# yflyl613/Tiny-NewsRec

Hardware: AMD Instinct MI355X
Metric: training impressions/sec (higher is better)
Workload: dtype fp16; 1 GPU; Tiny-NewsRec 4-layer student (train [2, 3]) + 4-teacher KD (title-emb MSE + soft-CE), fwd+bwd+AMSGrad; batch_per_gpu=32, global_batch=32, user_log_length=50, candidates=5, num_words_title=30, news_dim=256, n_news=51282, parallelism=dp1

## Files before the change

tiny-newsrec_amd/csrc/heads.hip:

```cpp
#include "common.h"

namespace {

__global__ __launch_bounds__(256) void attpool_long_score_kernel(const float* __restrict__ e, int64_t lde, const float* __restrict__ w2,
                                                                 const float* __restrict__ b2, int Q, float* __restrict__ alpha,
                                                                 int64_t n_tok, int L) {
    const int lane = threadIdx.x & 63;
    const int64_t t = (int64_t)blockIdx.x * 4 + (threadIdx.x >> 6);
    if (t >= n_tok) return;
    const float* er = e + t * lde;
    float s = 0.f;
    for (int q = lane; q < Q; q += 64) s += er[q] * w2[q];
    s = wave_sum(s);
    const int Lr = (L + 31) & ~31;
    if (lane == 0) alpha[(t / L) * Lr + (t % L)] = __expf(s + b2[0]);
}
__global__ __launch_bounds__(256) void attpool_long_fwd_fin_kernel(const float* __restrict__ ws, float* __restrict__ alpha,
                                                                   float* __restrict__ nv, float* __restrict__ den, int L, int H) {
    __shared__ float dsh, al[512];
    const int Lr = (L + 31) & ~31, nch = (L + AP_CH - 1) / AP_CH;
    const int64_t n = blockIdx.x;
    for (int i = threadIdx.x; i < L; i += 256) al[i] = alpha[n * Lr + i];
    __syncthreads();
    if (threadIdx.x == 0) {
        float d = 0.f;
        for (int i = 0; i < L; ++i) d += al[i];
        dsh = d + 1e-8f;
        den[n] = d + 1e-8f;
    }
    __syncthreads();
    const float d = dsh;
    for (int c = threadIdx.x * 4; c < H; c += 1024) {
        f32x4 a = *(const f32x4*)(ws + (n * nch) * H + c);
        for (int ch = 1; ch < nch; ++ch) a += *(const f32x4*)(ws + (n * nch + ch) * H + c);
        *(f32x4*)(nv + n * H + c) = a / d;
    }
    for (int i = threadIdx.x; i < Lr; i += 256) alpha[n * Lr + i] = i < L ? al[i] / d : 0.f;
}
__global__ __launch_bounds__(256) void attpool_long_bwd_fin_kernel(const float* __restrict__ part, int Q, int64_t lddpre, int nch,
                                                                   float* __restrict__ dw2_part, float* __restrict__ db2_part,
                                                                   float* __restrict__ db1_part) {
    const int64_t n = blockIdx.x;
    const int64_t W = Q + lddpre + 1;
    for (int64_t j = threadIdx.x; j < W; j += 256) {
        float s = part[(n * nch) * W + j];
        for (int ch = 1; ch < nch; ++ch) s += part[(n * nch + ch) * W + j];
        if (j < Q) dw2_part[n * Q + j] = s;
        else if (j < Q + lddpre) { if (db1_part) db1_part[n * lddpre + (j - Q)] = s; }
        else db2_part[n] = s;
    }
}

struct SgemmArgs {
    const float* A; int64_t a_rs, a_cs, sA;
    const float* B; int64_t b_rs, b_cs, sB;
    float* C; int64_t ldc, sC;
    const float* bias; int64_t sBias;
    int M, N, K;
    float alpha, beta;
    int ksplit, kchunk, batch;
    float* A_out;
};

constexpr int SG_BK = 64;
__device__ __forceinline__ void sgemm_tile(const SgemmArgs& g, int bx, int by, int bz, float (&As)[64][SG_BK + 1], float (&Bs)[64][SG_BK + 1]) {
    const int tid = threadIdx.x, lane = tid & 63, w = tid >> 6, wm = w >> 1, wn = w & 1;
    const int zb = bz / g.ksplit, zk = bz - zb * g.ksplit;
    const float* A = g.A + zb * g.sA;
    const float* B = g.B + zb * g.sB;
    float* C = g.ksplit > 1 ? g.C + ((int64_t)zk * g.batch + zb) * g.M * g.N : g.C + zb * g.sC;
    const int64_t ldc = g.ksplit > 1 ? g.N : g.ldc;
    const int m0 = by * 64, n0 = bx * 64;
    const int kbeg = zk * g.kchunk;
    const int kend = kbeg + g.kchunk < g.K ? kbeg + g.kchunk : g.K;
    f32x16 acc;
#pragma unroll
    for (int r = 0; r < 16; ++r) acc[r] = 0.f;
    const bool a_kfast = g.a_cs == 1, b_kfast = g.b_cs == 1;
    constexpr int NQ = 64 * SG_BK / 256;
    const int ra0 = a_kfast ? tid >> 6 : tid & 63, ka0 = a_kfast ? tid & 63 : tid >> 6;
    const int rb0 = b_kfast ? tid >> 6 : tid & 63, kb0 = b_kfast ? tid & 63 : tid >> 6;
    float av[NQ], bv[NQ];
    auto fetch = [&](int k0) {
#pragma unroll
        for (int q = 0; q < NQ; ++q) {
            const int ra = a_kfast ? ra0 + 4 * q : ra0, ka = a_kfast ? ka0 : ka0 + 4 * q;
            const int rb = b_kfast ? rb0 + 4 * q : rb0, kb = b_kfast ? kb0 : kb0 + 4 * q;
            av[q] = (m0 + ra < g.M && k0 + ka < kend) ? A[(int64_t)(m0 + ra) * g.a_rs + (int64_t)(k0 + ka) * g.a_cs] : 0.f;
            bv[q] = (n0 + rb < g.N && k0 + kb < kend) ? B[(int64_t)(n0 + rb) * g.b_rs + (int64_t)(k0 + kb) * g.b_cs] : 0.f;
        }
    };
    fetch(kbeg);
    for (int k0 = kbeg; k0 < kend; k0 += SG_BK) {
#pragma unroll
        for (int q = 0; q < NQ; ++q) {
            const int ra = a_kfast ? ra0 + 4 * q : ra0, ka = a_kfast ? ka0 : ka0 + 4 * q;
            const int rb = b_kfast ? rb0 + 4 * q : rb0, kb = b_kfast ? kb0 : kb0 + 4 * q;
            As[ra][ka] = av[q];
            Bs[rb][kb] = bv[q];
        }
        __syncthreads();
        if (k0 + SG_BK < kend) fetch(k0 + SG_BK);
        const int kk_end = kend - k0 < SG_BK ? kend - k0 : SG_BK;
        for (int kk = 0; kk < kk_end; kk += 2) {
            float a = As[wm * 32 + (lane & 31)][kk + (lane >> 5)];
            float b = Bs[wn * 32 + (lane & 31)][kk + (lane >> 5)];
            acc = __builtin_amdgcn_mfma_f32_32x32x2f32(a, b, acc, 0, 0, 0);
        }
        __syncthreads();
    }
    const int n = n0 + wn * 32 + (lane & 31);
    if (n >= g.N) return;
    const float bias = (g.bias && g.ksplit == 1) ? g.bias[zb * g.sBias + n] : 0.f;
#pragma unroll
    for (int r = 0; r < 16; ++r) {
        int m = m0 + wm * 32 + (r & 3) + 8 * (r >> 2) + 4 * (lane >> 5);
        if (m < g.M) {
            float* c = C + (int64_t)m * ldc + n;
            if (g.ksplit > 1) {
                *c = acc[r];
            } else {
                float v = g.alpha * acc[r] + bias;
                if (g.beta != 0.f) v += g.beta * *c;
                *c = v;
            }
        }
    }
}

__global__ __launch_bounds__(256) void sgemm_kernel(SgemmArgs g) {
    __shared__ float As[64][SG_BK + 1], Bs[64][SG_BK + 1];
    sgemm_tile(g, blockIdx.x, blockIdx.y, blockIdx.z, As, Bs);
}

constexpr int SG_MAXP = 8;
struct SgemmGroup {
    SgemmArgs a[SG_MAXP];
    int start[SG_MAXP + 1];
    int gx[SG_MAXP], gy[SG_MAXP];
    int64_t rstart[SG_MAXP + 1];
    float alpha[SG_MAXP], beta[SG_MAXP];
    int n;
};
__global__ __launch_bounds__(256) void sgemm_group_kernel(SgemmGroup g) {
    __shared__ float As[64][SG_BK + 1], Bs[64][SG_BK + 1];
    const int b = blockIdx.x;
    int i = 0;
#pragma unroll
    for (int k = 1; k < SG_MAXP; ++k)
        if (k < g.n && b >= g.start[k]) i = k;
    const int l = b - g.start[i];
    const int per = g.gx[i] * g.gy[i];
    const int bz = l / per, r = l - bz * per;
    const int by = r / g.gx[i], bx = r - by * g.gx[i];
    sgemm_tile(g.a[i], bx, by, bz, As, Bs);
}
__global__ __launch_bounds__(256) void sgemm_group_reduce_kernel(SgemmGroup g) {
    const int64_t e = (int64_t)blockIdx.x * blockDim.x + threadIdx.x;
    if (e >= g.rstart[g.n]) return;
    int i = 0;
#pragma unroll
    for (int k = 1; k < SG_MAXP; ++k)
        if (k < g.n && e >= g.rstart[k]) i = k;
    const SgemmArgs& a = g.a[i];
    const int64_t per = (int64_t)a.M * a.N, total = per * a.batch, j = e - g.rstart[i];
    const float* part = a.C;
    float t = part[j];
    for (int s = 1; s < a.ksplit; ++s) t += part[(int64_t)s * total + j];
    const int z = (int)(j / per);
    const int64_t rr = j - (int64_t)z * per;
    const int m = (int)(rr / a.N), n = (int)(rr - (int64_t)m * a.N);
    float* c = (float*)a.A_out + (int64_t)z * a.sC + (int64_t)m * a.ldc + n;
    float v = g.alpha[i] * t + (a.bias ? a.bias[(int64_t)z * a.sBias + n] : 0.f);
    if (g.beta[i] != 0.f) v += g.beta[i] * *c;
    *c = v;
}

__global__ __launch_bounds__(256) void sgemm_reduce_kernel(const float* __restrict__ part, int ksplit, int batch, int M, int N,
                                                           float* __restrict__ C, int64_t ldc, int64_t sC,
                                                           const float* __restrict__ bias, int64_t sBias, float alpha, float beta) {
    const int64_t per = (int64_t)M * N, total = per * batch;
    const int64_t i = (int64_t)blockIdx.x * blockDim.x + threadIdx.x;
    if (i >= total) return;
    float t = part[i];
    for (int s = 1; s < ksplit; ++s) t += part[(int64_t)s * total + i];
    const int z = (int)(i / per);
    const int64_t r = i - (int64_t)z * per;
    const int m = (int)(r / N), n = (int)(r - (int64_t)m * N);
    float* c = C + (int64_t)z * sC + (int64_t)m * ldc + n;
    float v = alpha * t + (bias ? bias[(int64_t)z * sBias + n] : 0.f);
    if (beta != 0.f) v += beta * *c;
    *c = v;
}

__global__ void gather_rows_kernel(const float* __restrict__ tbl, int64_t R, const int32_t* __restrict__ idx,
                                   int64_t n_idx, int D, float* __restrict__ out, int64_t out_rows, int64_t out_row0) {
    int64_t t = (int64_t)blockIdx.x * blockDim.x + threadIdx.x;
    int d4 = D / 4;
    int64_t total = n_idx * d4;
    if (t >= total) return;
    int z = blockIdx.y;
    int64_t r = t / d4;
    int c = (int)(t - r * d4) * 4;
    *(f32x4*)(out + ((int64_t)z * out_rows + out_row0 + r) * D + c) =
        *(const f32x4*)(tbl + ((int64_t)z * R + idx[r]) * D + c);
}


__global__ __launch_bounds__(1024) void segment_sum_rows_kernel(const float* __restrict__ src, const int32_t* __restrict__ order,
                                                                const int32_t* __restrict__ seg, int D, float* __restrict__ out) {
    extern __shared__ __attribute__((aligned(16))) float sm[];
    const int u = blockIdx.x, lane = threadIdx.x & 63, w = threadIdx.x >> 6;
    const int j0 = seg[u], j1 = seg[u + 1];
    if (j1 - j0 <= 4) {
        if (w == 0)
            for (int c = lane * 4; c < D; c += 256) {
                f32x4 a = (f32x4){0.f, 0.f, 0.f, 0.f};
                for (int j = j0; j < j1; ++j) a += *(const f32x4*)(src + (int64_t)order[j] * D + c);
                *(f32x4*)(out + (int64_t)u * D + c) = a;
            }
        return;
    }
    for (int c = lane * 4; c < D; c += 256) {
        f32x4 a[4];
#pragma unroll
        for (int q = 0; q < 4; ++q) a[q] = (f32x4){0.f, 0.f, 0.f, 0.f};
        int j = j0 + w;
        for (; j + 48 < j1; j += 64) {
// ... 635 lines not shown
    if (threadIdx.x == 0) {
        losses[0] = red[0][0] / (float)B;
        losses[1] = red[1][0] / (float)B;
    }
}

__global__ __launch_bounds__(256) void kd_embed_loss_kernel(const float* __restrict__ S, const float* __restrict__ P,
                                                            const float* __restrict__ tw, float* __restrict__ dS,
                                                            float* __restrict__ dP, float* __restrict__ part, int B,
                                                            int U, int C, int D, int T) {
    const int lane = threadIdx.x & 63;
    const int64_t wv = (int64_t)blockIdx.x * 4 + (threadIdx.x >> 6);
    const int64_t nh = (int64_t)B * U, nn = (int64_t)B * (U + C), rtot = nn + B;
    if (wv >= rtot) return;
    int b;
    float rowscale;
    if (wv < nh) { b = (int)(wv / U); rowscale = 1.f / (float)(U + C); }
    else if (wv < nn) { b = (int)((wv - nh) / C); rowscale = 1.f / (float)(U + C); }
    else { b = (int)(wv - nn); rowscale = 1.f; }
    float loss = 0.f;
    for (int c = lane * 4; c < D; c += 256) {
        f32x4 s = *(const f32x4*)(S + wv * D + c);
        f32x4 g = (f32x4){0.f, 0.f, 0.f, 0.f};
        for (int i = 0; i < T; ++i) {
            float wi = tw[(int64_t)b * T + i];
            float ci = wi * rowscale * 2.f / ((float)D * (float)B);
            int64_t off = ((int64_t)i * rtot + wv) * D + c;
            f32x4 df = s - *(const f32x4*)(P + off);
            loss += wi * rowscale * (df[0] * df[0] + df[1] * df[1] + df[2] * df[2] + df[3] * df[3]);
            g += ci * df;
            *(f32x4*)(dP + off) = -ci * df;
        }
        *(f32x4*)(dS + wv * D + c) = g;
    }
    loss = wave_sum(loss);
    if (lane == 0) part[wv] = loss / ((float)D * (float)B);
}

__global__ __launch_bounds__(256) void score_bwd_kernel(const float* __restrict__ vec, const int32_t* __restrict__ cidx,
                                                        const float* __restrict__ user, const float* __restrict__ dscore,
                                                        float* __restrict__ dvec, float* __restrict__ duser, int C, int D) {
    const int b = blockIdx.x;
    for (int d = threadIdx.x; d < D; d += 256) {
        float u = user[(int64_t)b * D + d], acc = 0.f;
        for (int c = 0; c < C; ++c) {
            float g = dscore[(int64_t)b * C + c];
            int64_t row = cidx[(int64_t)b * C + c];
            acc += g * vec[row * D + d];
            dvec[row * D + d] += g * u;
        }
        duser[(int64_t)b * D + d] += acc;
    }
}

}

void attpool_long_score_launch(const float* e, int64_t lde, const float* w2, const float* b2, int Q, float* alpha, int64_t n_tok,
                               int L, hipStream_t st) {
    hipLaunchKernelGGL(attpool_long_score_kernel, dim3((unsigned)((n_tok + 3) / 4)), dim3(256), 0, st, e, lde, w2, b2, Q, alpha, n_tok, L);
}
void attpool_long_fwd_fin_launch(const float* ws, float* alpha, float* nv, float* den, int64_t n_seq, int L, int H, hipStream_t st) {
    hipLaunchKernelGGL(attpool_long_fwd_fin_kernel, dim3((unsigned)n_seq), dim3(256), 0, st, ws, alpha, nv, den, L, H);
}
void attpool_long_bwd_fin_launch(const float* part, int Q, int64_t lddpre, int nch, float* dw2_part, float* db2_part,
                                 float* db1_part, int64_t n_seq, hipStream_t st) {
    hipLaunchKernelGGL(attpool_long_bwd_fin_kernel, dim3((unsigned)n_seq), dim3(256), 0, st, part, Q, lddpre, nch, dw2_part,
                       db2_part, db1_part);
}

extern "C" int tnr_sgemm(const float* A, int64_t a_rs, int64_t a_cs, int64_t sA, const int32_t* a_idx, const float* B,
                         int64_t b_rs, int64_t b_cs, int64_t sB, float* C, int64_t ldc, int64_t sC, const float* bias,
                         int64_t sBias, int64_t M, int64_t N, int64_t K, int batch, float alpha, float beta,
                         int ksplit, float* part, void* stream) {
    TNR_CHECK_ARG(A && B && C && M >= 1 && N >= 1 && K >= 1 && batch >= 1, "tnr_sgemm: bad argument");
    TNR_CHECK_ARG(a_idx == nullptr, "tnr_sgemm: row gather is done by tnr_gather_rows");
    if (ksplit < 1) ksplit = 1;
    int kchunk = (int)K;
    if (ksplit > 1) {
        TNR_CHECK_ARG(part != nullptr, "tnr_sgemm: split-K needs the partial buffer (ksplit * batch * M * N floats)");
        kchunk = (int)(((K + ksplit - 1) / ksplit + 15) / 16 * 16);
        ksplit = (int)((K + kchunk - 1) / kchunk);
    }
    SgemmArgs g{A, a_rs, a_cs, sA, B, b_rs, b_cs, sB, ksplit > 1 ? part : C, ldc, sC, bias, sBias, (int)M, (int)N, (int)K,
                alpha, ksplit > 1 ? 0.f : beta, ksplit, kchunk, batch, C};
    dim3 grid((unsigned)((N + 63) / 64), (unsigned)((M + 63) / 64), (unsigned)(batch * ksplit));
    hipLaunchKernelGGL(sgemm_kernel, grid, dim3(256), 0, (hipStream_t)stream, g);
    TNR_CHECK_LAUNCH("tnr_sgemm");
    if (ksplit > 1) {
        const int64_t total = (int64_t)batch * M * N;
        hipLaunchKernelGGL(sgemm_reduce_kernel, dim3((unsigned)((total + 255) / 256)), dim3(256), 0, (hipStream_t)stream, part,
                           ksplit, batch, (int)M, (int)N, C, ldc, sC, bias, sBias, alpha, beta);
        TNR_CHECK_LAUNCH("tnr_sgemm/reduce");
    }
    return TNR_OK;
}

extern "C" int tnr_sgemm_group(const tnr_sgemm_problem_t* p, int n, void* stream) {
    TNR_CHECK_ARG(p && n >= 1 && n <= SG_MAXP, "tnr_sgemm_group: 1..%d problems", SG_MAXP);
    SgemmGroup g;
    g.n = n;
    g.start[0] = 0;
    g.rstart[0] = 0;
    for (int i = 0; i < n; ++i) {
        const tnr_sgemm_problem_t& q = p[i];
        TNR_CHECK_ARG(q.A && q.B && q.C && q.M >= 1 && q.N >= 1 && q.K >= 1 && q.batch >= 1, "tnr_sgemm_group: bad problem %d", i);
        int ksplit = q.ksplit < 1 ? 1 : q.ksplit;
        int kchunk = (int)q.K;
        if (ksplit > 1) {
            TNR_CHECK_ARG(q.part != nullptr, "tnr_sgemm_group: split-K needs the partial buffer (problem %d)", i);
            kchunk = (int)(((q.K + ksplit - 1) / ksplit + 15) / 16 * 16);
            ksplit = (int)((q.K + kchunk - 1) / kchunk);
        }
        g.a[i] = SgemmArgs{q.A, q.a_rs, q.a_cs, q.sA, q.B, q.b_rs, q.b_cs, q.sB, ksplit > 1 ? q.part : q.C, q.ldc, q.sC, q.bias, q.sBias,
                           (int)q.M, (int)q.N, (int)q.K, q.alpha, ksplit > 1 ? 0.f : q.beta, ksplit, kchunk, q.batch, q.C};
        g.gx[i] = (int)((q.N + 63) / 64);
        g.gy[i] = (int)((q.M + 63) / 64);
        g.start[i + 1] = g.start[i] + g.gx[i] * g.gy[i] * q.batch * ksplit;
        g.rstart[i + 1] = g.rstart[i] + (ksplit > 1 ? (int64_t)q.batch * q.M * q.N : 0);
        g.alpha[i] = q.alpha;
        g.beta[i] = q.beta;
    }
    for (int i = n; i < SG_MAXP; ++i) { g.start[i + 1] = g.start[n]; g.rstart[i + 1] = g.rstart[n]; g.gx[i] = g.gy[i] = 1; g.a[i] = g.a[0]; g.alpha[i] = g.beta[i] = 0.f; }
    hipLaunchKernelGGL(sgemm_group_kernel, dim3((unsigned)g.start[n]), dim3(256), 0, (hipStream_t)stream, g);
    TNR_CHECK_LAUNCH("tnr_sgemm_group");
    if (g.rstart[n] > 0) {
        hipLaunchKernelGGL(sgemm_group_reduce_kernel, dim3((unsigned)((g.rstart[n] + 255) / 256)), dim3(256), 0, (hipStream_t)stream, g);
        TNR_CHECK_LAUNCH("tnr_sgemm_group/reduce");
    }
    return TNR_OK;
}

__global__ __launch_bounds__(256) void concat_i32_kernel(const int32_t* __restrict__ a, int64_t na, const int32_t* __restrict__ b,
                                                         int64_t nb, int32_t* __restrict__ out) {
    const int64_t i = (int64_t)blockIdx.x * blockDim.x + threadIdx.x;
    if (i < na) out[i] = a[i];
    else if (i < na + nb) out[i] = b[i - na];
}

extern "C" int tnr_concat_i32(const int32_t* a, int64_t na, const int32_t* b, int64_t nb, int32_t* out, void* stream) {
    TNR_CHECK_ARG(out && na >= 0 && nb >= 0 && na + nb >= 1 && (a || na == 0) && (b || nb == 0), "tnr_concat_i32: bad argument");
    hipLaunchKernelGGL(concat_i32_kernel, dim3((unsigned)((na + nb + 255) / 256)), dim3(256), 0, (hipStream_t)stream, a, na, b, nb, out);
    TNR_CHECK_LAUNCH("tnr_concat_i32");
    return TNR_OK;
}

extern "C" int tnr_gather_rows(const float* tbl, int64_t R, const int32_t* idx, int64_t n_idx, int D, int n_model,
                               float* out, int64_t out_rows, int64_t out_row0, void* stream) {
    TNR_CHECK_ARG(tbl && idx && out && n_idx >= 1 && (D % 4) == 0 && n_model >= 1, "tnr_gather_rows: bad argument");
    int64_t total = n_idx * (D / 4);
    dim3 grid((unsigned)((total + 255) / 256), (unsigned)n_model);
    hipLaunchKernelGGL(gather_rows_kernel, grid, dim3(256), 0, (hipStream_t)stream, tbl, R, idx, n_idx, D, out, out_rows,
                       out_row0);
    TNR_CHECK_LAUNCH("tnr_gather_rows");
    return TNR_OK;
}

extern "C" int tnr_segment_sum_rows(const float* src, const int32_t* order, const int32_t* seg, int64_t n_seg, int D,
                                    float* out, void* stream) {
    TNR_CHECK_ARG(src && order && seg && out && n_seg >= 1 && D >= 4 && (D % 4) == 0 && D <= 2048,
                  "tnr_segment_sum_rows: bad argument");
    hipLaunchKernelGGL(segment_sum_rows_kernel, dim3((unsigned)n_seg), dim3(1024), 16 * D * sizeof(float),
                       (hipStream_t)stream, src, order, seg, D, out);
    TNR_CHECK_LAUNCH("tnr_segment_sum_rows");
    return TNR_OK;
}

extern "C" int tnr_scatter_sum_rows(const float* src, int64_t n, int D, const int32_t* keys_sorted, const int32_t* order,
                                    int32_t skip_key, float* table, int64_t table_rows, int accumulate, void* stream) {
    TNR_CHECK_ARG(src && keys_sorted && order && table && n >= 1 && n <= 0x7FFFFFFF && table_rows >= 1 && D >= 4 && (D % 4) == 0 &&
                  D <= 2048, "tnr_scatter_sum_rows: bad argument");
    hipLaunchKernelGGL(scatter_sum_rows_kernel, dim3((unsigned)n), dim3(1024), 16 * D * sizeof(float), (hipStream_t)stream, src, n,
                       D, keys_sorted, order, skip_key, table, table_rows, accumulate);
    TNR_CHECK_LAUNCH("tnr_scatter_sum_rows");
    return TNR_OK;
}

static int user_shape_ok(int B, int U, int C, int D, int Q) {
    return B >= 1 && U >= 1 && U <= MAXU && C >= 0 && (D % 4) == 0 && D >= 4 && Q >= 4 && (Q % 4) == 0;
}

extern "C" int tnr_user_score_fwd(const float* vec, int64_t R, const int32_t* hidx, const int32_t* cidx,
                                  const float* mask, const float* pad, const float* w1, const float* b1, const float* w2,
                                  const float* b2, int user_log_mask, const float* epre, const float* epad, float* user,
                                  int64_t user_stride,
                                  float* score, float* e, float* alpha, float* den, int n_model, int B, int U, int C, int D,
                                  int Q, void* stream) {
    TNR_CHECK_ARG(vec && hidx && cidx && mask && pad && w1 && b1 && w2 && b2 && user && score && e && alpha && den,
                  "tnr_user_score_fwd: null pointer");
    TNR_CHECK_ARG(user_shape_ok(B, U, C, D, Q) && n_model >= 1 && user_stride >= (int64_t)B * D,
                  "tnr_user_score_fwd: bad shape (U <= %d)", MAXU);
    if (!epre) {
        size_t lf = sizeof(float) * ((size_t)64 * (D + UF_XTRA) + (size_t)U * Q + MAXU + D);
        TNR_CHECK_ARG((D % 8) == 0 && lf <= 160 * 1024, "tnr_user_score_fwd: fused fc1 needs D %% 8 == 0 and 64 (D + 4) + U Q floats of LDS");
        TNR_ONCE_PER_DEVICE({
            (void)hipFuncSetAttribute((const void*)user_fwd_fused_kernel, hipFuncAttributeMaxDynamicSharedMemorySize, 160 * 1024);
        });
        hipLaunchKernelGGL(user_fwd_fused_kernel, dim3((unsigned)B, (unsigned)n_model), dim3(UF_THREADS), lf, (hipStream_t)stream,
// ... 133 lines not shown
```

tiny-newsrec_amd/csrc/testhooks.hip:

```cpp
#include "common.h"

namespace {
__global__ __launch_bounds__(1024) void cu_hog_kernel(unsigned long long ticks) {
    extern __shared__ char hog_lds[];
    if (threadIdx.x == 0) hog_lds[0] = 1;
    const unsigned long long t0 = __builtin_amdgcn_s_memrealtime();
    while (__builtin_amdgcn_s_memrealtime() - t0 < ticks) __builtin_amdgcn_s_sleep(64);
}
}

void tnr_set_error(const char*, ...) {}

extern "C" int tnr_debug_cu_hog(int n_wg, int us, void* stream) {
    if (!(n_wg >= 1 && n_wg <= 1024 && us >= 0 && us <= 100000)) return TNR_EINVAL;
    TNR_ONCE_PER_DEVICE({ (void)hipFuncSetAttribute((const void*)cu_hog_kernel, hipFuncAttributeMaxDynamicSharedMemorySize, 160 * 1024); });
    hipLaunchKernelGGL(cu_hog_kernel, dim3((unsigned)n_wg), dim3(1024), 160 * 1024, (hipStream_t)stream, (unsigned long long)us * 100ull);
    return hipGetLastError() == hipSuccess ? TNR_OK : TNR_ELAUNCH;
}
```

tiny-newsrec_amd/tnr_hip.py:

```python
import ctypes
import os

import torch

_HERE = os.path.dirname(os.path.abspath(__file__))
LIB_PATH = os.path.join(_HERE, "csrc", "libtnr_hip.so")

BF16, F16, F32 = 0, 1, 2
ROUTE_128, ROUTE_256x128, ROUTE_256, ROUTE_224 = 128, 2128, 256, 224
EPI_BIAS, EPI_GELU, EPI_TANH, EPI_RES, EPI_MULDGELU, EPI_OUTF32, EPI_AUXOUT, EPI_COLSUM = 1, 2, 4, 8, 16, 32, 64, 128

_c = ctypes
_P, _I, _L, _F = _c.c_void_p, _c.c_int, _c.c_int64, _c.c_float

DROP_EMB, DROP_PROB, DROP_ATTN_OUT, DROP_FFN_OUT = 0, 1, 2, 3


class Dropout(_c.Structure):
    _fields_ = [("seed", _c.c_uint64), ("site", _c.c_uint32), ("call", _c.c_uint32), ("p", _c.c_double)]

    @classmethod
    def site_of(cls, p, seed, kind, layer, call):
        if p is None or p <= 0.0:
            return None
# ... 91 lines not shown
    "tnr_attn_l32_bwd": [_P, _P, _P, _P, _P, _P, _L, _I, _I, _P],
    "tnr_attn_long_fwd": [_P, _P, _P, _P, _P, _L, _I, _I, _P],
    "tnr_attn_long_bwd": [_P, _P, _P, _P, _P, _P, _P, _P, _L, _I, _I, _P],
    "tnr_colsum": [_P, _L, _I, _L, _L, _P, _P, _I, _P],
    "tnr_colsum_batched": [_P, _L, _L, _I, _L, _L, _I, _P, _P, _I, _P],
    "tnr_colsum_part_elems": [_L, _L],
    "tnr_attpool_fwd": [_P, _P, _L, _P, _P, _I, _P, _P, _P, _L, _I, _I, _P],
    "tnr_attpool_bwd": [_P, _P, _L, _P, _I, _P, _P, _P, _P, _P, _L, _P, _P, _P, _L, _I, _I, _P],
    "tnr_attpool_fwd_long": [_P, _P, _L, _P, _P, _I, _P, _P, _P, _P, _L, _I, _I, _P],
    "tnr_attpool_bwd_long": [_P, _P, _L, _P, _I, _P, _P, _P, _P, _L, _P, _P, _P, _P, _L, _I, _I, _P],
    "tnr_sgemm": [_P, _L, _L, _L, _P, _P, _L, _L, _L, _P, _L, _L, _P, _L, _L, _L, _L, _I, _F, _F, _I, _P, _P],
    "tnr_sgemm_group": [_c.POINTER(SgemmProblem), _I, _P],
    "tnr_gemm_tn_wgrad_group": [_c.POINTER(WgradProblem), _I, _P],
    "tnr_concat_i32": [_P, _L, _P, _L, _P, _P],
    "tnr_gather_rows": [_P, _L, _P, _L, _I, _I, _P, _L, _L, _P],
    "tnr_segment_sum_rows": [_P, _P, _P, _L, _I, _P, _P],
    "tnr_scatter_sum_rows": [_P, _L, _I, _P, _P, _I, _P, _L, _I, _P],
    "tnr_user_score_fwd": [_P, _L, _P, _P, _P, _P, _P, _P, _P, _P, _I, _P, _P, _P, _L, _P, _P, _P, _P, _I, _I, _I, _I, _I, _I, _P],
    "tnr_user_bwd_pre": [_P, _P, _P, _P, _P, _I, _P, _P, _P, _P, _P, _P, _I, _I, _I, _I, _P],
    "tnr_user_bwd_post": [_P, _P, _P, _P, _P, _I, _P, _P, _I, _I, _I, _I, _P],
    "tnr_user_bwd_part_stride": [_I, _I],
    "tnr_user_blend_fwd": [_P, _L, _P, _P, _P, _I, _P, _I, _I, _I, _I, _P],
    "tnr_user_blend_bwd": [_P, _P, _P, _I, _P, _P, _L, _I, _I, _I, _P],
    "tnr_nrms_attn_fwd": [_P, _P, _I, _P, _L, _I, _I, _I, _I, _P],
    "tnr_nrms_attn_bwd": [_P, _P, _I, _P, _P, _I, _I, _I, _P],
    "tnr_score_bwd": [_P, _P, _P, _P, _P, _P, _I, _I, _I, _P],
    "tnr_kd_score_loss": [_P, _P, _P, _F, _F, _P, _P, _P, _I, _I, _I, _P],
    "tnr_kd_embed_loss": [_P, _P, _P, _P, _P, _P, _P, _I, _I, _I, _I, _I, _P],
    "tnr_reduce_rows": [_P, _L, _L, _L, _P, _I, _P],
    "tnr_reduce_multi": [_P, _I, _P],
    "tnr_dropout_mask": [_D, _L, _L, _P, _P],
    "tnr_dropout_mask_probs": [_D, _L, _I, _I, _P, _P],
    "tnr_dropout_mask_split": [_D, _D, _L, _L, _L, _P, _P],
    "tnr_scale_inplace": [_P, _L, _F, _P],
    "tnr_amsgrad_step": [_P, _P, _P, _P, _P, _L, _I, _F, _F, _F, _F, _F, _P],
    "tnr_amsgrad_step_guarded": [_P, _P, _P, _P, _P, _L, _I, _F, _F, _F, _F, _F, _P, _c.c_uint, _c.c_uint, _P],
    "tnr_grad_nonfinite": [_P, _L, _P, _c.c_uint, _P],
    "tnr_grad_nonfinite_scan": [_P, _L, _P, _c.c_uint, _P],
    "tnr_grad_nonfinite_commit": [_P, _c.c_uint, _P],
    "tnr_refresh_shadows": [_P, _I, _L, _P, _P],
    "tnr_cast_f32_to_bf16": [_P, _P, _L, _P],
    "tnr_cast_bf16_to_f32": [_P, _P, _L, _P],
}
TYPED = ["tnr_embed_ln_fwd", "tnr_embed_ln_fwd_indexed", "tnr_embed_ln_bwd", "tnr_embed_ln_bwd_indexed", "tnr_gemm_nt", "tnr_gemm_nt_ex", "tnr_gemm_colsum_rows", "tnr_gemm_nt_route",
         "tnr_gemm_tn_wgrad", "tnr_gemm_tn_wgrad_ex", "tnr_gemm_tn_wgrad_group", "tnr_gemm_tn_ws_elems", "tnr_ln_fwd", "tnr_ln_bwd", "tnr_attn_l32_fwd", "tnr_attn_l32_bwd", "tnr_attn_long_fwd", "tnr_attn_long_bwd",
         "tnr_colsum", "tnr_colsum_batched", "tnr_attpool_fwd", "tnr_attpool_bwd", "tnr_attpool_fwd_long", "tnr_attpool_bwd_long", "tnr_attpool_long_ws_elems", "tnr_refresh_shadows",
         "tnr_cast_f32_to_bf16", "tnr_cast_bf16_to_f32", "tnr_pool_fwd", "tnr_pool_bwd"]
for _n in ("tnr_embed_ln_fwd", "tnr_embed_ln_fwd_indexed", "tnr_attn_l32_fwd", "tnr_attn_l32_bwd", "tnr_attn_long_fwd", "tnr_attn_long_bwd"):
    _SIG[_n + "_do"] = _SIG[_n][:-1] + [_D] + ([_P] if "embed" in _n else []) + [_P]
    TYPED.append(_n + "_do")
_SIG["tnr_gemm_nt_do"] = _SIG["tnr_gemm_nt_ex"][:-1] + [_D, _P]
_SIG["tnr_ln_bwd_do"] = _SIG["tnr_ln_bwd"][:-1] + [_P, _D, _P]
_SIG["tnr_gemm_nt_do_split"] = _SIG["tnr_gemm_nt_do"][:-1] + [_D, _L, _P]
_SIG["tnr_ln_bwd_do_split"] = _SIG["tnr_ln_bwd_do"][:-1] + [_D, _L, _P]
TYPED += ["tnr_gemm_nt_do", "tnr_ln_bwd_do", "tnr_gemm_nt_do_split", "tnr_ln_bwd_do_split"]
for _n in TYPED:
    _SIG[_n + "_f16"] = _SIG[_n]
_RET = {"tnr_attpool_long_ws_elems": _L, "tnr_attpool_long_ws_elems_f16": _L, "tnr_gemm_tn_ws_elems": _L, "tnr_gemm_tn_ws_elems_f16": _L, "tnr_gemm_colsum_rows_f16": _L, "tnr_gemm_colsum_rows": _L, "tnr_ln_bwd_part_elems": _L, "tnr_ln_bwd_blocks": _L, "tnr_embed_ln_bwd_part_elems": _L, "tnr_embed_ln_bwd_blocks": _L, "tnr_colsum_part_elems": _L,
        "tnr_user_bwd_part_stride": _L}
EXPORTS = sorted(_SIG) + ["tnr_last_error"]

_lib = None


class TnrError(RuntimeError):
    pass


def lib():
    global _lib
    if _lib is None:
        if not os.path.exists(LIB_PATH):
            raise TnrError("libtnr_hip.so not built: run `make -C tiny-newsrec_amd/csrc` (or __graft_entry__.build())")
        L = ctypes.CDLL(LIB_PATH)
        for name, args in _SIG.items():
            fn = getattr(L, name)
            fn.argtypes = args
            fn.restype = _RET.get(name, _I)
        L.tnr_last_error.restype = ctypes.c_char_p
        _lib = L
    return _lib


def _ptr(t):
    if t is None:
        return None
    if isinstance(t, int):
        return t
    return t.data_ptr()


def _conv(a):
    if isinstance(a, Dropout):
        return ctypes.byref(a)
    return _ptr(a) if (isinstance(a, torch.Tensor) or a is None) else a


_raw_stream = getattr(torch._C, "_cuda_getCurrentRawStream", None)


def stream():
    if _raw_stream is not None:
        return _raw_stream(torch.cuda.current_device())
    return torch.cuda.current_stream().cuda_stream


TIMED = {}
TIMED_ALL = None


def _all_begin():
    if TIMED_ALL is None:
        return None
    e0 = torch.cuda.Event(enable_timing=True)
    e0.record()
    return e0


def _all_end(e0, name):
    if e0 is not None:
        e1 = torch.cuda.Event(enable_timing=True)
        e1.record()
        TIMED_ALL.append((e0, e1, name))


def _work(name, conv):
    if name.startswith("tnr_gemm_nt"):
        return 2.0 * conv[6] * conv[7] * conv[8]
    if name.startswith("tnr_gemm_tn_wgrad"):
        return 2.0 * conv[6] * conv[7] * conv[8]
    return 0.0


def call(name, *args):
    L = lib()
    conv = [_conv(a) for a in args]
    rec = TIMED.get(name)
    if rec is not None or TIMED_ALL is not None:
        e0, e1 = torch.cuda.Event(enable_timing=True), torch.cuda.Event(enable_timing=True)
        e0.record()
    rc = getattr(L, name)(*conv, stream())
    if rec is not None:
        e1.record()
        rec.append((e0, e1, _work(name, conv), (conv[6], conv[7], conv[8], conv[14]) if "gemm_nt" in name else None))
    elif TIMED_ALL is not None:
        e1.record()
        TIMED_ALL.append((e0, e1, name))
    if rc != 0:
        raise TnrError("%s failed (%d): %s" % (name, rc, L.tnr_last_error().decode()))


def query(name, *args):
    return getattr(lib(), name)(*args)
```

Baseline: 4364 impressions/s.

## Double-buffer fp32 sgemm tiles with vectorized swizzled LDS staging

```diff
diff --git a/tiny-newsrec_amd/csrc/heads.hip b/tiny-newsrec_amd/csrc/heads.hip
--- a/tiny-newsrec_amd/csrc/heads.hip
+++ b/tiny-newsrec_amd/csrc/heads.hip
@@ -60,53 +60,130 @@
     float alpha, beta;
     int ksplit, kchunk, batch;
     float* A_out;
+    int a_mode, b_mode;
 };
 
-constexpr int SG_BK = 64;
-__device__ __forceinline__ void sgemm_tile(const SgemmArgs& g, int bx, int by, int bz, float (&As)[64][SG_BK + 1], float (&Bs)[64][SG_BK + 1]) {
+constexpr int SG_BK = 32;
+constexpr int SG_STAGE = 64 * SG_BK;
+enum { SG_VEC_K = 0, SG_VEC_ROW = 1, SG_SCALAR = 2 };
+
+__device__ __forceinline__ int sg_at(int k, int r) { return k * 64 + ((((r >> 2) ^ ((k >> 2) & 7)) << 2) | (r & 3)); }
+
+typedef __attribute__((ext_vector_type(2))) float f32x2;
+__device__ __forceinline__ int sg_fresh(int tid) { asm volatile("" : "+v"(tid)); return tid; }
+
+template <int mode> struct SgOperand {
+    const float* X; int64_t rs, cs;
+    int r0, R;
+    f32x4 v[2];
+    __device__ __forceinline__ void fetch(int tid, int k0, int kend) {
+#pragma unroll
+        for (int q = 0; q < 2; ++q) {
+            if (mode == SG_VEC_K) {
+                const int r = r0 + 2 * (tid >> 3) + q, kk = k0 + 4 * (tid & 7);
+                v[q] = *(const f32x4*)(r < R && kk < kend ? X + (int64_t)r * rs + kk : X);
+            } else if (mode == SG_VEC_ROW) {
+                const int r = r0 + 4 * (tid & 15), kk = k0 + (tid >> 4) + 16 * q;
+                v[q] = *(const f32x4*)(r < R && kk < kend ? X + (int64_t)kk * cs + r : X);
+            } else {
+                const int ts = sg_fresh(tid);
+#pragma unroll
+                for (int e = 0; e < 4; ++e) {
+                    const int r = r0 + (cs == 1 ? (ts >> 5) + 8 * (4 * q + e) : ts & 63);
+                    const int kk = k0 + (cs == 1 ? ts & 31 : (ts >> 6) + 4 * (4 * q + e));
+                    v[q][e] = *(r < R && kk < kend ? X + (int64_t)r * rs + (int64_t)kk * cs : X);
+                }
+            }
+        }
+    }
+    __device__ __forceinline__ void stash(int tid, float* S, int k0, int kend) const {
+        if (mode == SG_VEC_K) {
+            const int lo = tid & 7, hi = tid >> 3;
+#pragma unroll
+            for (int j = 0; j < 4; ++j) {
+                f32x2 o;
+#pragma unroll
+                for (int q = 0; q < 2; ++q) o[q] = (r0 + 2 * hi + q < R && k0 + 4 * lo + j < kend) ? v[q][j] : 0.f;
+                *(f32x2*)&S[sg_at(4 * lo + j, 2 * hi)] = o;
+            }
+        } else if (mode == SG_VEC_ROW) {
+            const int lo = tid & 15, hi = tid >> 4;
+#pragma unroll
+            for (int q = 0; q < 2; ++q) {
+                f32x4 o;
+#pragma unroll
+                for (int e = 0; e < 4; ++e) o[e] = (r0 + 4 * lo + e < R && k0 + hi + 16 * q < kend) ? v[q][e] : 0.f;
+                *(f32x4*)&S[sg_at(hi + 16 * q, 4 * lo)] = o;
+            }
+        } else {
+            const int ts = sg_fresh(tid);
+#pragma unroll
+            for (int q = 0; q < 2; ++q)
+#pragma unroll
+                for (int e = 0; e < 4; ++e) {
+                    const int r = cs == 1 ? (ts >> 5) + 8 * (4 * q + e) : ts & 63;
+                    const int k = cs == 1 ? ts & 31 : (ts >> 6) + 4 * (4 * q + e);
+                    S[sg_at(k, r)] = (r0 + r < R && k0 + k < kend) ? v[q][e] : 0.f;
+                }
+        }
+    }
+};
+
+inline int sg_mode(const float* X, int64_t rs, int64_t cs, int64_t sX) {
+    const bool al = ((uintptr_t)X & 15) == 0 && (sX & 3) == 0;
+    if (cs == 1) return al && (rs & 3) == 0 ? SG_VEC_K : SG_SCALAR;
+    if (rs == 1) return al && (cs & 3) == 0 ? SG_VEC_ROW : SG_SCALAR;
+    return SG_SCALAR;
+}
+
+template <int AM, int BM>
+__device__ __forceinline__ void sgemm_tile_on(const SgemmArgs& g, int bx, int by, int bz, float* As, float* Bs) {
     const int tid = threadIdx.x, lane = tid & 63, w = tid >> 6, wm = w >> 1, wn = w & 1;
     const int zb = bz / g.ksplit, zk = bz - zb * g.ksplit;
-    const float* A = g.A + zb * g.sA;
-    const float* B = g.B + zb * g.sB;
     float* C = g.ksplit > 1 ? g.C + ((int64_t)zk * g.batch + zb) * g.M * g.N : g.C + zb * g.sC;
     const int64_t ldc = g.ksplit > 1 ? g.N : g.ldc;
     const int m0 = by * 64, n0 = bx * 64;
     const int kbeg = zk * g.kchunk;
     const int kend = kbeg + g.kchunk < g.K ? kbeg + g.kchunk : g.K;
+    const int nsteps = (kend - kbeg + SG_BK - 1) / SG_BK;
     f32x16 acc;
 #pragma unroll
     for (int r = 0; r < 16; ++r) acc[r] = 0.f;
-    const bool a_kfast = g.a_cs == 1, b_kfast = g.b_cs == 1;
-    constexpr int NQ = 64 * SG_BK / 256;
-    const int ra0 = a_kfast ? tid >> 6 : tid & 63, ka0 = a_kfast ? tid & 63 : tid >> 6;
-    const int rb0 = b_kfast ? tid >> 6 : tid & 63, kb0 = b_kfast ? tid & 63 : tid >> 6;
-    float av[NQ], bv[NQ];
-    auto fetch = [&](int k0) {
-#pragma unroll
-        for (int q = 0; q < NQ; ++q) {
-            const int ra = a_kfast ? ra0 + 4 * q : ra0, ka = a_kfast ? ka0 : ka0 + 4 * q;
-            const int rb = b_kfast ? rb0 + 4 * q : rb0, kb = b_kfast ? kb0 : kb0 + 4 * q;
-            av[q] = (m0 + ra < g.M && k0 + ka < kend) ? A[(int64_t)(m0 + ra) * g.a_rs + (int64_t)(k0 + ka) * g.a_cs] : 0.f;
-            bv[q] = (n0 + rb < g.N && k0 + kb < kend) ? B[(int64_t)(n0 + rb) * g.b_rs + (int64_t)(k0 + kb) * g.b_cs] : 0.f;
+    SgOperand<AM> oa;
+    SgOperand<BM> ob;
+    oa.X = g.A + zb * g.sA; oa.rs = g.a_rs; oa.cs = g.a_cs; oa.r0 = m0; oa.R = g.M;
+    ob.X = g.B + zb * g.sB; ob.rs = g.b_rs; ob.cs = g.b_cs; ob.r0 = n0; ob.R = g.N;
+    const int ra = wm * 32 + (lane & 31), rb = wn * 32 + (lane & 31), h = lane >> 5;
+    auto stage = [&](int s) {
+        oa.stash(tid, As + (s & 1) * SG_STAGE, kbeg + s * SG_BK, kend);
+        ob.stash(tid, Bs + (s & 1) * SG_STAGE, kbeg + s * SG_BK, kend);
+        if (s + 1 < nsteps) {
+            oa.fetch(tid, kbeg + (s + 1) * SG_BK, kend);
+            ob.fetch(tid, kbeg + (s + 1) * SG_BK, kend);
         }
     };
-    fetch(kbeg);
-    for (int k0 = kbeg; k0 < kend; k0 += SG_BK) {
-#pragma unroll
-        for (int q = 0; q < NQ; ++q) {
-            const int ra = a_kfast ? ra0 + 4 * q : ra0, ka = a_kfast ? ka0 : ka0 + 4 * q;
-            const int rb = b_kfast ? rb0 + 4 * q : rb0, kb = b_kfast ? kb0 : kb0 + 4 * q;
-            As[ra][ka] = av[q];
-            Bs[rb][kb] = bv[q];
-        }
-        __syncthreads();
-        if (k0 + SG_BK < kend) fetch(k0 + SG_BK);
-        const int kk_end = kend - k0 < SG_BK ? kend - k0 : SG_BK;
-        for (int kk = 0; kk < kk_end; kk += 2) {
-            float a = As[wm * 32 + (lane & 31)][kk + (lane >> 5)];
-            float b = Bs[wn * 32 + (lane & 31)][kk + (lane >> 5)];
-            acc = __builtin_amdgcn_mfma_f32_32x32x2f32(a, b, acc, 0, 0, 0);
-        }
+    oa.fetch(tid, kbeg, kend);
+    ob.fetch(tid, kbeg, kend);
+    stage(0);
+    __syncthreads();
+    for (int s = 0; s < nsteps; ++s) {
+        if (s > 0 && s + 1 < nsteps) stage(s + 1);
+        const float* Ac = As + (s & 1) * SG_STAGE;
+        const float* Bc = Bs + (s & 1) * SG_STAGE;
+        const int left = kend - (kbeg + s * SG_BK);
+        if (left >= SG_BK) {
+#pragma unroll
+            for (int kk = 0; kk < SG_BK; kk += 2) {
+                const int x = ((kk >> 2) & 7) << 2;
+                acc = __builtin_amdgcn_mfma_f32_32x32x2f32(Ac[(kk + h) * 64 + (ra ^ x)], Bc[(kk + h) * 64 + (rb ^ x)], acc, 0, 0, 0);
+            }
+        } else {
+            for (int kk = 0; kk < left; kk += 2) {
+                const int x = ((kk >> 2) & 7) << 2;
+                acc = __builtin_amdgcn_mfma_f32_32x32x2f32(Ac[(kk + h) * 64 + (ra ^ x)], Bc[(kk + h) * 64 + (rb ^ x)], acc, 0, 0, 0);
+            }
+        }
+        if (s == 0 && nsteps > 1) stage(1);
         __syncthreads();
     }
     const int n = n0 + wn * 32 + (lane & 31);
@@ -128,8 +205,18 @@
     }
 }
 
-__global__ __launch_bounds__(256) void sgemm_kernel(SgemmArgs g) {
-    __shared__ float As[64][SG_BK + 1], Bs[64][SG_BK + 1];
+__device__ __forceinline__ void sgemm_tile(const SgemmArgs& g, int bx, int by, int bz, float* As, float* Bs) {
+    switch (g.a_mode * 3 + g.b_mode) {
+#define TNR_SG_CASE(a, b) case a * 3 + b: sgemm_tile_on<a, b>(g, bx, by, bz, As, Bs); break;
+        TNR_SG_CASE(0, 0) TNR_SG_CASE(0, 1) TNR_SG_CASE(0, 2)
+        TNR_SG_CASE(1, 0) TNR_SG_CASE(1, 1) TNR_SG_CASE(1, 2)
+        TNR_SG_CASE(2, 0) TNR_SG_CASE(2, 1) TNR_SG_CASE(2, 2)
+#undef TNR_SG_CASE
+    }
+}
+
+__global__ __launch_bounds__(256, 4) void sgemm_kernel(SgemmArgs g) {
+    __shared__ __attribute__((aligned(16))) float As[2 * SG_STAGE], Bs[2 * SG_STAGE];
     sgemm_tile(g, blockIdx.x, blockIdx.y, blockIdx.z, As, Bs);
 }
 
@@ -142,8 +229,8 @@
     float alpha[SG_MAXP], beta[SG_MAXP];
     int n;
 };
-__global__ __launch_bounds__(256) void sgemm_group_kernel(SgemmGroup g) {
-    __shared__ float As[64][SG_BK + 1], Bs[64][SG_BK + 1];
+__global__ __launch_bounds__(256, 4) void sgemm_group_kernel(SgemmGroup g) {
+    __shared__ __attribute__((aligned(16))) float As[2 * SG_STAGE], Bs[2 * SG_STAGE];
     const int b = blockIdx.x;
     int i = 0;
 #pragma unroll
@@ -945,7 +1032,7 @@
         ksplit = (int)((K + kchunk - 1) / kchunk);
     }
     SgemmArgs g{A, a_rs, a_cs, sA, B, b_rs, b_cs, sB, ksplit > 1 ? part : C, ldc, sC, bias, sBias, (int)M, (int)N, (int)K,
-                alpha, ksplit > 1 ? 0.f : beta, ksplit, kchunk, batch, C};
+                alpha, ksplit > 1 ? 0.f : beta, ksplit, kchunk, batch, C, sg_mode(A, a_rs, a_cs, sA), sg_mode(B, b_rs, b_cs, sB)};
     dim3 grid((unsigned)((N + 63) / 64), (unsigned)((M + 63) / 64), (unsigned)(batch * ksplit));
     hipLaunchKernelGGL(sgemm_kernel, grid, dim3(256), 0, (hipStream_t)stream, g);
     TNR_CHECK_LAUNCH("tnr_sgemm");
@@ -964,18 +1051,29 @@
     g.n = n;
     g.start[0] = 0;
     g.rstart[0] = 0;
+    int order[SG_MAXP], steps[SG_MAXP];
     for (int i = 0; i < n; ++i) {
-        const tnr_sgemm_problem_t& q = p[i];
-        TNR_CHECK_ARG(q.A && q.B && q.C && q.M >= 1 && q.N >= 1 && q.K >= 1 && q.batch >= 1, "tnr_sgemm_group: bad problem %d", i);
+        TNR_CHECK_ARG(p[i].K >= 1, "tnr_sgemm_group: bad problem %d", i);
+        const int ks = p[i].ksplit < 1 ? 1 : p[i].ksplit;
+        const int64_t kc = ks > 1 ? ((p[i].K + ks - 1) / ks + 15) / 16 * 16 : p[i].K;
+        steps[i] = (int)(((kc < p[i].K ? kc : p[i].K) + SG_BK - 1) / SG_BK);
+        int j = i;
+        for (; j > 0 && steps[order[j - 1]] < steps[i]; --j) order[j] = order[j - 1];
+        order[j] = i;
+    }
+    for (int i = 0; i < n; ++i) {
+        const tnr_sgemm_problem_t& q = p[order[i]];
+        TNR_CHECK_ARG(q.A && q.B && q.C && q.M >= 1 && q.N >= 1 && q.K >= 1 && q.batch >= 1, "tnr_sgemm_group: bad problem %d", order[i]);
         int ksplit = q.ksplit < 1 ? 1 : q.ksplit;
         int kchunk = (int)q.K;
         if (ksplit > 1) {
-            TNR_CHECK_ARG(q.part != nullptr, "tnr_sgemm_group: split-K needs the partial buffer (problem %d)", i);
+            TNR_CHECK_ARG(q.part != nullptr, "tnr_sgemm_group: split-K needs the partial buffer (problem %d)", order[i]);
             kchunk = (int)(((q.K + ksplit - 1) / ksplit + 15) / 16 * 16);
             ksplit = (int)((q.K + kchunk - 1) / kchunk);
         }
         g.a[i] = SgemmArgs{q.A, q.a_rs, q.a_cs, q.sA, q.B, q.b_rs, q.b_cs, q.sB, ksplit > 1 ? q.part : q.C, q.ldc, q.sC, q.bias, q.sBias,
-                           (int)q.M, (int)q.N, (int)q.K, q.alpha, ksplit > 1 ? 0.f : q.beta, ksplit, kchunk, q.batch, q.C};
+                           (int)q.M, (int)q.N, (int)q.K, q.alpha, ksplit > 1 ? 0.f : q.beta, ksplit, kchunk, q.batch, q.C,
+                           sg_mode(q.A, q.a_rs, q.a_cs, q.sA), sg_mode(q.B, q.b_rs, q.b_cs, q.sB)};
         g.gx[i] = (int)((q.N + 63) / 64);
         g.gy[i] = (int)((q.M + 63) / 64);
         g.start[i + 1] = g.start[i] + g.gx[i] * g.gy[i] * q.batch * ksplit;
diff --git a/tiny-newsrec_amd/csrc/testhooks.hip b/tiny-newsrec_amd/csrc/testhooks.hip
--- a/tiny-newsrec_amd/csrc/testhooks.hip
+++ b/tiny-newsrec_amd/csrc/testhooks.hip
@@ -17,3 +17,132 @@
     hipLaunchKernelGGL(cu_hog_kernel, dim3((unsigned)n_wg), dim3(1024), 160 * 1024, (hipStream_t)stream, (unsigned long long)us * 100ull);
     return hipGetLastError() == hipSuccess ? TNR_OK : TNR_ELAUNCH;
 }
+
+namespace {
+struct SgemmArgs {
+    const float* A; int64_t a_rs, a_cs, sA;
+    const float* B; int64_t b_rs, b_cs, sB;
+    float* C; int64_t ldc, sC;
+    const float* bias; int64_t sBias;
+    int M, N, K;
+    float alpha, beta;
+    int ksplit, kchunk, batch;
+    float* A_out;
+};
+
+constexpr int SG_BK = 64;
+__device__ __forceinline__ void sgemm_tile(const SgemmArgs& g, int bx, int by, int bz, float (&As)[64][SG_BK + 1], float (&Bs)[64][SG_BK + 1]) {
+    const int tid = threadIdx.x, lane = tid & 63, w = tid >> 6, wm = w >> 1, wn = w & 1;
+    const int zb = bz / g.ksplit, zk = bz - zb * g.ksplit;
+    const float* A = g.A + zb * g.sA;
+    const float* B = g.B + zb * g.sB;
+    float* C = g.ksplit > 1 ? g.C + ((int64_t)zk * g.batch + zb) * g.M * g.N : g.C + zb * g.sC;
+    const int64_t ldc = g.ksplit > 1 ? g.N : g.ldc;
+    const int m0 = by * 64, n0 = bx * 64;
+    const int kbeg = zk * g.kchunk;
+    const int kend = kbeg + g.kchunk < g.K ? kbeg + g.kchunk : g.K;
+    f32x16 acc;
+#pragma unroll
+    for (int r = 0; r < 16; ++r) acc[r] = 0.f;
+    const bool a_kfast = g.a_cs == 1, b_kfast = g.b_cs == 1;
+    constexpr int NQ = 64 * SG_BK / 256;
+    const int ra0 = a_kfast ? tid >> 6 : tid & 63, ka0 = a_kfast ? tid & 63 : tid >> 6;
+    const int rb0 = b_kfast ? tid >> 6 : tid & 63, kb0 = b_kfast ? tid & 63 : tid >> 6;
+    float av[NQ], bv[NQ];
+    auto fetch = [&](int k0) {
+#pragma unroll
+        for (int q = 0; q < NQ; ++q) {
+            const int ra = a_kfast ? ra0 + 4 * q : ra0, ka = a_kfast ? ka0 : ka0 + 4 * q;
+            const int rb = b_kfast ? rb0 + 4 * q : rb0, kb = b_kfast ? kb0 : kb0 + 4 * q;
+            av[q] = (m0 + ra < g.M && k0 + ka < kend) ? A[(int64_t)(m0 + ra) * g.a_rs + (int64_t)(k0 + ka) * g.a_cs] : 0.f;
+            bv[q] = (n0 + rb < g.N && k0 + kb < kend) ? B[(int64_t)(n0 + rb) * g.b_rs + (int64_t)(k0 + kb) * g.b_cs] : 0.f;
+        }
+    };
+    fetch(kbeg);
+    for (int k0 = kbeg; k0 < kend; k0 += SG_BK) {
+#pragma unroll
+        for (int q = 0; q < NQ; ++q) {
+            const int ra = a_kfast ? ra0 + 4 * q : ra0, ka = a_kfast ? ka0 : ka0 + 4 * q;
+            const int rb = b_kfast ? rb0 + 4 * q : rb0, kb = b_kfast ? kb0 : kb0 + 4 * q;
+            As[ra][ka] = av[q];
+            Bs[rb][kb] = bv[q];
+        }
+        __syncthreads();
+        if (k0 + SG_BK < kend) fetch(k0 + SG_BK);
+        const int kk_end = kend - k0 < SG_BK ? kend - k0 : SG_BK;
+        for (int kk = 0; kk < kk_end; kk += 2) {
+            float a = As[wm * 32 + (lane & 31)][kk + (lane >> 5)];
+            float b = Bs[wn * 32 + (lane & 31)][kk + (lane >> 5)];
+            acc = __builtin_amdgcn_mfma_f32_32x32x2f32(a, b, acc, 0, 0, 0);
+        }
+        __syncthreads();
+    }
+    const int n = n0 + wn * 32 + (lane & 31);
+    if (n >= g.N) return;
+    const float bias = (g.bias && g.ksplit == 1) ? g.bias[zb * g.sBias + n] : 0.f;
+#pragma unroll
+    for (int r = 0; r < 16; ++r) {
+        int m = m0 + wm * 32 + (r & 3) + 8 * (r >> 2) + 4 * (lane >> 5);
+        if (m < g.M) {
+            float* c = C + (int64_t)m * ldc + n;
+            if (g.ksplit > 1) {
+                *c = acc[r];
+            } else {
+                float v = g.alpha * acc[r] + bias;
+                if (g.beta != 0.f) v += g.beta * *c;
+                *c = v;
+            }
+        }
+    }
+}
+
+__global__ __launch_bounds__(256) void sgemm_kernel(SgemmArgs g) {
+    __shared__ float As[64][SG_BK + 1], Bs[64][SG_BK + 1];
+    sgemm_tile(g, blockIdx.x, blockIdx.y, blockIdx.z, As, Bs);
+}
+
+__global__ __launch_bounds__(256) void sgemm_reduce_kernel(const float* __restrict__ part, int ksplit, int batch, int M, int N,
+                                                           float* __restrict__ C, int64_t ldc, int64_t sC,
+                                                           const float* __restrict__ bias, int64_t sBias, float alpha, float beta) {
+    const int64_t per = (int64_t)M * N, total = per * batch;
+    const int64_t i = (int64_t)blockIdx.x * blockDim.x + threadIdx.x;
+    if (i >= total) return;
+    float t = part[i];
+    for (int s = 1; s < ksplit; ++s) t += part[(int64_t)s * total + i];
+    const int z = (int)(i / per);
+    const int64_t r = i - (int64_t)z * per;
+    const int m = (int)(r / N), n = (int)(r - (int64_t)m * N);
+    float* c = C + (int64_t)z * sC + (int64_t)m * ldc + n;
+    float v = alpha * t + (bias ? bias[(int64_t)z * sBias + n] : 0.f);
+    if (beta != 0.f) v += beta * *c;
+    *c = v;
+}
+
+}
+
+extern "C" int tnr_debug_sgemm_one_buffer(const float* A, int64_t a_rs, int64_t a_cs, int64_t sA, const int32_t* a_idx, const float* B,
+                         int64_t b_rs, int64_t b_cs, int64_t sB, float* C, int64_t ldc, int64_t sC, const float* bias,
+                         int64_t sBias, int64_t M, int64_t N, int64_t K, int batch, float alpha, float beta,
+                         int ksplit, float* part, void* stream) {
+    TNR_CHECK_ARG(A && B && C && M >= 1 && N >= 1 && K >= 1 && batch >= 1, "tnr_debug_sgemm_one_buffer: bad argument");
+    TNR_CHECK_ARG(a_idx == nullptr, "tnr_debug_sgemm_one_buffer: row gather is done by tnr_gather_rows");
+    if (ksplit < 1) ksplit = 1;
+    int kchunk = (int)K;
+    if (ksplit > 1) {
+        TNR_CHECK_ARG(part != nullptr, "tnr_debug_sgemm_one_buffer: split-K needs the partial buffer (ksplit * batch * M * N floats)");
+        kchunk = (int)(((K + ksplit - 1) / ksplit + 15) / 16 * 16);
+        ksplit = (int)((K + kchunk - 1) / kchunk);
+    }
+    SgemmArgs g{A, a_rs, a_cs, sA, B, b_rs, b_cs, sB, ksplit > 1 ? part : C, ldc, sC, bias, sBias, (int)M, (int)N, (int)K,
+                alpha, ksplit > 1 ? 0.f : beta, ksplit, kchunk, batch, C};
+    dim3 grid((unsigned)((N + 63) / 64), (unsigned)((M + 63) / 64), (unsigned)(batch * ksplit));
+    hipLaunchKernelGGL(sgemm_kernel, grid, dim3(256), 0, (hipStream_t)stream, g);
+    TNR_CHECK_LAUNCH("tnr_debug_sgemm_one_buffer");
+    if (ksplit > 1) {
+        const int64_t total = (int64_t)batch * M * N;
+        hipLaunchKernelGGL(sgemm_reduce_kernel, dim3((unsigned)((total + 255) / 256)), dim3(256), 0, (hipStream_t)stream, part,
+                           ksplit, batch, (int)M, (int)N, C, ldc, sC, bias, sBias, alpha, beta);
+        TNR_CHECK_LAUNCH("tnr_debug_sgemm_one_buffer/reduce");
+    }
+    return TNR_OK;
+}
diff --git a/tiny-newsrec_amd/tnr_hip.py b/tiny-newsrec_amd/tnr_hip.py
--- a/tiny-newsrec_amd/tnr_hip.py
+++ b/tiny-newsrec_amd/tnr_hip.py
@@ -197,6 +197,20 @@
     return _lib
 
 
+_hooks = None
+
+
+def testhooks():
+    global _hooks
+    if _hooks is None:
+        L = ctypes.CDLL(os.path.join(os.path.dirname(LIB_PATH), "libtnr_testhooks.so"))
+        L.tnr_debug_cu_hog.argtypes = [_I, _I, _P]
+        L.tnr_debug_sgemm_one_buffer.argtypes = _SIG["tnr_sgemm"]
+        L.tnr_debug_cu_hog.restype = L.tnr_debug_sgemm_one_buffer.restype = _I
+        _hooks = L
+    return _hooks
+
+
 def _ptr(t):
     if t is None:
         return None
```

Result: no change. 4385 impressions/s, median of 6 (+0.5%).
